# duyhominhnguyen/conan-fgw

Measured on AMD Instinct MI355X. Metric: molecules/s (K=5 conformers), higher is better.
Workload: dtype f32

## Files before the change

### conan-fgw_amd/csrc/filter_fused.hip

```cpp
#include "fp_planes.h"

namespace {

constexpr int GP = 64;
constexpr int W1S = GP + 8;
constexpr int FF_THREADS = 512;

constexpr int FF_NPL = 2;
constexpr int FF_OP = 36;

template <int F, bool CF = false, int NT = FF_THREADS>
__global__ void __launch_bounds__(NT) k_filter_fused(
    const float *__restrict__ dist, const int *__restrict__ num_edges_dev, int max_edges, const float *__restrict__ offset,
    int Gs, float coeff, float cutoff, const float *__restrict__ w1, const float *__restrict__ b1,
    const float *__restrict__ w2, const float *__restrict__ b2, float *__restrict__ Wout, float *__restrict__ h1_out,
    const float *__restrict__ xin = nullptr, const int *__restrict__ col = nullptr, const int *__restrict__ tgt = nullptr) {
    constexpr int MB = F / 32;
    constexpr int W2S = F + 8;
    constexpr int W2WORDS = (FF_NPL * F * W2S) / 2;
    extern __shared__ __attribute__((aligned(16))) float lds[];
    constexpr int W1WORDS = (FF_NPL * F * W1S) / 2;
    float *W1L = lds;
    float *W2L = W1L + W1WORDS;
    float *B1L = W2L + W2WORDS;
    float *B2L = B1L + F;
    float *OFL = B2L + F;
    float *OT = OFL + GP + (threadIdx.x >> 6) * (32 * FF_OP);
    __shared__ float wred[NT / 64];
    float us1 = 1.0f, us2 = 1.0f;
    const int tid = threadIdx.x, lane = tid & 63, wave = tid >> 6;
    const int E = num_edges_dev ? min(*num_edges_dev, max_edges) : max_edges;
    const int tiles = (E + 31) >> 5;
    if (!CF && (int)blockIdx.x * (NT / 64) >= tiles) return;
    if (CF && tiles == 0) return;

    {
        constexpr int PER1 = (F * GP + NT - 1) / NT;
        float wv[PER1];
#pragma unroll
        for (int u = 0; u < PER1; ++u) {
            const int t = tid + u * NT, f = t / GP, k = t - f * GP;
            wv[u] = (t < F * GP && k < Gs) ? w1[(size_t)f * Gs + k] : 0.f;
        }
        float sc1 = 1.0f;
        float am = 0.f;
#pragma unroll
        for (int u = 0; u < PER1; ++u) am = fmaxf(am, fabsf(wv[u]));
        __syncthreads();
        pow2_scale(block_absmax<NT>(am, wred), sc1, us1);
#pragma unroll
        for (int u = 0; u < PER1; ++u) {
            const int t = tid + u * NT, f = t / GP, k = t - f * GP;
            if (t >= F * GP) continue;
            _Float16 *W1H = reinterpret_cast<_Float16 *>(W1L);
            const float v = wv[u] * sc1;
            const _Float16 h1 = (_Float16)v;
            W1H[(0 * F + f) * W1S + k] = h1;
            W1H[(1 * F + f) * W1S + k] = (_Float16)(v - (float)h1);
        }
    }
    {
        constexpr int PER2 = (F * F + NT - 1) / NT;
        float wv[PER2];
#pragma unroll
        for (int u = 0; u < PER2; ++u) { const int t = tid + u * NT; wv[u] = t < F * F ? w2[t] : 0.f; }
        float sc2 = 1.0f;
        float am = 0.f;
#pragma unroll
        for (int u = 0; u < PER2; ++u) am = fmaxf(am, fabsf(wv[u]));
        __syncthreads();
        pow2_scale(block_absmax<NT>(am, wred), sc2, us2);
#pragma unroll
        for (int u = 0; u < PER2; ++u) {
            const int t = tid + u * NT;
            if (t >= F * F) continue;
            const int f2 = t / F, f = t - f2 * F;
            const int kk = f & 15, hh = (kk >> 2) & 1, jj = (kk & 3) + 4 * (kk >> 3);
            const int colp = (f & ~15) + 8 * hh + jj;
            _Float16 *W2H = reinterpret_cast<_Float16 *>(W2L);
            const float v = wv[u] * sc2;
            const _Float16 h1 = (_Float16)v;
            W2H[(0 * F + f2) * W2S + colp] = h1;
            W2H[(1 * F + f2) * W2S + colp] = (_Float16)(v - (float)h1);
        }
    }
    for (int t = tid; t < F; t += NT) { B1L[t] = b1[t]; B2L[t] = b2[t]; }
    for (int t = tid; t < GP; t += NT) OFL[t] = t < Gs ? offset[t] : 0.f;
    __syncthreads();

    const int l31 = lane & 31, h = lane >> 5;
    const int per_wg = CF ? (tiles + (int)gridDim.x - 1) / (int)gridDim.x : 0;
    const int lb = CF ? ((gridDim.x & 7) == 0 ? xcd_contiguous_block((int)blockIdx.x, (int)gridDim.x) : (int)blockIdx.x) : 0;
    const int t_begin = CF ? lb * per_wg + wave : blockIdx.x * (NT / 64) + wave;
    const int t_end = CF ? min(tiles, (lb + 1) * per_wg) : tiles;
    const int wave_stride = CF ? NT / 64 : gridDim.x * (NT / 64);
    for (int tile = t_begin; tile < t_end; tile += wave_stride) {
        const int e = (tile << 5) + l31;
        const bool valid = e < E;
        const float d = valid ? dist[e] : 0.f;
        int src = 0, trg = -1;
        if constexpr (CF) { if (valid) { src = col[e]; trg = tgt[e]; } }

        f32x16 acc1[MB];
#pragma unroll
        for (int mb = 0; mb < MB; ++mb)
#pragma unroll
            for (int r = 0; r < 16; ++r) acc1[mb][r] = 0.f;
        {
#pragma unroll
            for (int s = 0; s < GP / 16; ++s) {
                const int kb = 16 * s + 8 * h;
                const float4 o0 = *reinterpret_cast<const float4 *>(&OFL[kb]), o1 = *reinterpret_cast<const float4 *>(&OFL[kb + 4]);
                const float of[8] = {o0.x, o0.y, o0.z, o0.w, o1.x, o1.y, o1.z, o1.w};
                float rb[8];
#pragma unroll
                for (int j = 0; j < 8; ++j) { const float t0 = d - of[j]; rb[j] = exp_neg_f(coeff * (t0 * t0)); }
                const _Float16 *W1H = reinterpret_cast<const _Float16 *>(W1L);
                f16x8 q1, q2;
                split2h(rb, q1, q2);
#pragma unroll
                for (int mb = 0; mb < MB; ++mb) {
                    const int row = 32 * mb + l31;
                    const f16x8 p1 = *reinterpret_cast<const f16x8 *>(&W1H[(0 * F + row) * W1S + kb]);
                    const f16x8 p2 = *reinterpret_cast<const f16x8 *>(&W1H[(1 * F + row) * W1S + kb]);
                    acc1[mb] = __builtin_amdgcn_mfma_f32_32x32x16_f16(p2, q1, acc1[mb], 0, 0, 0);
                    acc1[mb] = __builtin_amdgcn_mfma_f32_32x32x16_f16(p1, q2, acc1[mb], 0, 0, 0);
                    acc1[mb] = __builtin_amdgcn_mfma_f32_32x32x16_f16(p1, q1, acc1[mb], 0, 0, 0);
                }
                __builtin_amdgcn_sched_barrier(0);
            }
        }
#pragma unroll
        for (int mb = 0; mb < MB; ++mb)
#pragma unroll
            for (int q = 0; q < 4; ++q) {
                const float4 bb = *reinterpret_cast<const float4 *>(&B1L[32 * mb + 8 * q + 4 * h]);
                const float us = us1;
                acc1[mb][4 * q + 0] = ssp_f(fmaf(acc1[mb][4 * q + 0], us, bb.x));
                acc1[mb][4 * q + 1] = ssp_f(fmaf(acc1[mb][4 * q + 1], us, bb.y));
                acc1[mb][4 * q + 2] = ssp_f(fmaf(acc1[mb][4 * q + 2], us, bb.z));
                acc1[mb][4 * q + 3] = ssp_f(fmaf(acc1[mb][4 * q + 3], us, bb.w));
            }
        if (!CF && h1_out) {
            typedef float f4 __attribute__((ext_vector_type(4)));
#pragma unroll
            for (int mb = 0; mb < MB; ++mb) {
#pragma unroll
                for (int q = 0; q < 4; ++q)
                    *reinterpret_cast<float4 *>(&OT[l31 * FF_OP + 8 * q + 4 * h]) =
                        make_float4(acc1[mb][4 * q], acc1[mb][4 * q + 1], acc1[mb][4 * q + 2], acc1[mb][4 * q + 3]);
                wave_lds_fence();
#pragma unroll
                for (int i = 0; i < 4; ++i) {
                    const int r = 8 * i + (lane >> 3), c = 4 * (lane & 7);
                    const float4 o = *reinterpret_cast<const float4 *>(&OT[r * FF_OP + c]);
                    const f4 hv4 = {o.x, o.y, o.z, o.w};
                    if ((tile << 5) + r < E) __builtin_nontemporal_store(hv4, reinterpret_cast<f4 *>(h1_out + (size_t)((tile << 5) + r) * F + 32 * mb + c));
                }
                wave_lds_fence();
            }
        }

        const float C = 0.5f * (cosf(__fdiv_rn(d * 3.14159265358979323846f, cutoff)) + 1.0f);
        constexpr int NG = MB >= 4 ? 2 : MB;
#pragma unroll
        for (int n0 = 0; n0 < MB; n0 += NG) {
            f32x16 acc2[NG];
#pragma unroll
            for (int nb = 0; nb < NG; ++nb)
#pragma unroll
                for (int r = 0; r < 16; ++r) acc2[nb][r] = 0.f;
            float4 xg[CF ? NG : 1][4];
            if constexpr (CF) {
#pragma unroll
                for (int nb = 0; nb < NG; ++nb)
#pragma unroll
                    for (int q = 0; q < 4; ++q)
                        xg[nb][q] = valid ? *reinterpret_cast<const float4 *>(xin + (size_t)src * F + 32 * (n0 + nb) + 8 * q + 4 * h) : make_float4(0.f, 0.f, 0.f, 0.f);
            }
            {
#pragma unroll
                for (int ms = 0; ms < 2 * MB; ++ms) {
                    const int mb = ms >> 1, sgrp = ms & 1;
                    float hv[8];
#pragma unroll
                    for (int j = 0; j < 8; ++j) hv[j] = acc1[mb][8 * sgrp + j];
                    const int colp = 32 * mb + 16 * sgrp + 8 * h;
                    const _Float16 *W2H = reinterpret_cast<const _Float16 *>(W2L);
                    f16x8 q1, q2;
                    split2h(hv, q1, q2);
#pragma unroll
                    for (int nb = 0; nb < NG; ++nb) {
                        const int row = 32 * (n0 + nb) + l31;
                        const f16x8 p1 = *reinterpret_cast<const f16x8 *>(&W2H[(0 * F + row) * W2S + colp]);
                        const f16x8 p2 = *reinterpret_cast<const f16x8 *>(&W2H[(1 * F + row) * W2S + colp]);
                        acc2[nb] = __builtin_amdgcn_mfma_f32_32x32x16_f16(p2, q1, acc2[nb], 0, 0, 0);
                        acc2[nb] = __builtin_amdgcn_mfma_f32_32x32x16_f16(p1, q2, acc2[nb], 0, 0, 0);
                        acc2[nb] = __builtin_amdgcn_mfma_f32_32x32x16_f16(p1, q1, acc2[nb], 0, 0, 0);
                    }
                    __builtin_amdgcn_sched_barrier(0);
                }
            }
#pragma unroll
            for (int nb = 0; nb < NG; ++nb) {
#pragma unroll
                for (int q = 0; q < 4; ++q) {
                    const float4 bb = *reinterpret_cast<const float4 *>(&B2L[32 * (n0 + nb) + 8 * q + 4 * h]);
                    float4 o;
                    const float us = us2;
                    o.x = fmaf(acc2[nb][4 * q + 0], us, bb.x) * C;
                    o.y = fmaf(acc2[nb][4 * q + 1], us, bb.y) * C;
                    o.z = fmaf(acc2[nb][4 * q + 2], us, bb.z) * C;
                    o.w = fmaf(acc2[nb][4 * q + 3], us, bb.w) * C;
                    if constexpr (CF) { o.x *= xg[nb][q].x; o.y *= xg[nb][q].y; o.z *= xg[nb][q].z; o.w *= xg[nb][q].w; }
                    *reinterpret_cast<float4 *>(&OT[l31 * FF_OP + 8 * q + 4 * h]) = o;
                }
                wave_lds_fence();
                if constexpr (CF) {
                    {
                        const int c = lane & 31, r0 = 16 * h;
                        float *ocol = Wout + 32 * (n0 + nb) + c;
                        const int t0 = __shfl(trg, 0, 64), t15 = __shfl(trg, 15, 64), t16 = __shfl(trg, 16, 64);
                        const bool joined = t15 == t16;
                        float accs = 0.f, carry = 0.f;
                        int cur = h ? t16 : t0;
                        bool first = true;
#pragma unroll
                        for (int r = 0; r < 16; ++r) {
                            const int tl = __shfl(trg, r, 64), th = __shfl(trg, 16 + r, 64);
                            const int tr = h ? th : tl;
                            if (tr != cur) {
                                if (h && first && joined) carry = accs;
                                else if (cur >= 0) unsafeAtomicAdd(ocol + (size_t)cur * F, accs);
                                accs = 0.f; cur = tr; first = false;
                            }
                            accs += OT[(r0 + r) * FF_OP + c];
                        }
                        if (h && first && joined) { carry = accs; cur = -1; }
                        const float down = __shfl(carry, (lane & 31) + 32, 64);
                        if (!h && joined) accs += down;
                        if (cur >= 0) unsafeAtomicAdd(ocol + (size_t)cur * F, accs);
                    }
                    wave_lds_fence();
                    continue;
                }
#pragma unroll
                for (int i = 0; i < 4; ++i) {
                    const int r = 8 * i + (lane >> 3), c = 4 * (lane & 7);
                    const float4 o = *reinterpret_cast<const float4 *>(&OT[r * FF_OP + c]);
                    if ((tile << 5) + r < E) *reinterpret_cast<float4 *>(Wout + (size_t)((tile << 5) + r) * F + 32 * (n0 + nb) + c) = o;
                }
                wave_lds_fence();
            }
        }
    }
}

template <int F, int NT>
int launch_nt(const float *dist, const int *num_edges_dev, int max_edges, const float *offset, int Gs, float coeff,
              float cutoff, const float *w1, const float *b1, const float *w2, const float *b2, float *W, float *h1, hipStream_t s) {
    const size_t lds = ((size_t)(FF_NPL * F * W1S) / 2 + (size_t)(FF_NPL * F * (F + 8)) / 2 + 2 * F + GP + (NT / 64) * 32 * FF_OP) * 4;
    (void)hipFuncSetAttribute(reinterpret_cast<const void *>(&k_filter_fused<F, false, NT>), hipFuncAttributeMaxDynamicSharedMemorySize, (int)lds);
    const int tiles = (max_edges + 31) / 32;
    int grid = (tiles + NT / 64 - 1) / (NT / 64);
    if (grid > 256) grid = 256;
    k_filter_fused<F, false, NT><<<grid, NT, lds, s>>>(dist, num_edges_dev, max_edges, offset, Gs, coeff, cutoff, w1, b1, w2, b2, W, h1);
    return hipGetLastError() == hipSuccess ? CONAN_OK : CONAN_E_LAUNCH;
}
template <int F>
int launch(const float *dist, const int *num_edges_dev, int max_edges, const float *offset, int Gs, float coeff,
           float cutoff, const float *w1, const float *b1, const float *w2, const float *b2, float *W, float *h1,
           hipStream_t s) {
    return launch_nt<F, FF_THREADS>(dist, num_edges_dev, max_edges, offset, Gs, coeff, cutoff, w1, b1, w2, b2, W, h1, s);
}

template <int F>
int launch_cf(const float *x, const float *dist, const int *col, const int *tgt, const int *num_edges_dev, int max_edges, const float *offset, int Gs,
              float coeff, float cutoff, const float *w1, const float *b1, const float *w2, const float *b2, int num_atoms, float *out, hipStream_t s) {
    const size_t lds = ((size_t)(FF_NPL * F * W1S) / 2 + (size_t)(FF_NPL * F * (F + 8)) / 2 + 2 * F + GP + (FF_THREADS / 64) * 32 * FF_OP) * 4;
    (void)hipFuncSetAttribute(reinterpret_cast<const void *>(&k_filter_fused<F, true>), hipFuncAttributeMaxDynamicSharedMemorySize, (int)lds);
    if (hipMemsetAsync(out, 0, (size_t)num_atoms * F * sizeof(float), s) != hipSuccess) return CONAN_E_LAUNCH;
    k_filter_fused<F, true><<<256, FF_THREADS, lds, s>>>(dist, num_edges_dev, max_edges, offset, Gs, coeff, cutoff, w1, b1, w2, b2, out, nullptr, x, col, tgt);
    return hipGetLastError() == hipSuccess ? CONAN_OK : CONAN_E_LAUNCH;
}

}

extern "C" {

int conan_filter_cfconv_fwd_supported(int num_gaussians, int num_filters) { return (num_gaussians >= 2 && num_gaussians <= GP && num_filters == 128) ? 1 : 0; }

int conan_filter_cfconv_fwd(const float *x, const float *dist, const int *col, const int *tgt, const int *num_edges_dev, int max_edges,
                            const float *offset, int num_gaussians, float coeff, float cutoff, int num_filters, const float *w1,
                            const float *b1, const float *w2, const float *b2, int num_atoms, float *out, void *stream) {
    if (!x || !dist || !col || !tgt || !offset || !w1 || !b1 || !w2 || !b2 || !out || max_edges < 0 || num_atoms < 0) return CONAN_E_BADARG;
    if (!conan_filter_cfconv_fwd_supported(num_gaussians, num_filters)) return CONAN_E_UNSUPPORTED;
    if (num_atoms == 0) return CONAN_OK;
    hipStream_t s = as_stream(stream);
    if (max_edges == 0) return hipMemsetAsync(out, 0, (size_t)num_atoms * num_filters * sizeof(float), s) == hipSuccess ? CONAN_OK : CONAN_E_LAUNCH;
    return launch_cf<128>(x, dist, col, tgt, num_edges_dev, max_edges, offset, num_gaussians, coeff, cutoff, w1, b1, w2, b2, num_atoms, out, s);
}

int conan_filter_fused_supported(int num_gaussians, int num_filters) {
    return (num_gaussians >= 2 && num_gaussians <= GP && (num_filters == 32 || num_filters == 64 || num_filters == 128)) ? 1 : 0;
}

int conan_filter_fwd(const float *dist, const int *num_edges_dev, int max_edges, const float *offset, int num_gaussians,
                     float coeff, float cutoff, int num_filters, const float *w1, const float *b1, const float *w2,
                     const float *b2, float *W, float *h1_out, void *stream) {
    if (!dist || !offset || !w1 || !b1 || !w2 || !b2 || !W || max_edges < 0) return CONAN_E_BADARG;
    if (!conan_filter_fused_supported(num_gaussians, num_filters)) return CONAN_E_UNSUPPORTED;
    if (max_edges == 0) return CONAN_OK;
    hipStream_t s = as_stream(stream);
#define CONAN_FF(FV) return launch<FV>(dist, num_edges_dev, max_edges, offset, num_gaussians, coeff, cutoff, w1, b1, w2, b2, W, h1_out, s)
    switch (num_filters) {
        case 32: CONAN_FF(32);
        case 64: CONAN_FF(64);
        default: CONAN_FF(128);
    }
#undef CONAN_FF
}

}
```

Before: 117,000.

## Software-pipeline filter kernel: overlap GEMM1, ssp, GEMM2 and next-tile Gaussians

```diff
diff --git a/conan-fgw_amd/csrc/filter_fused.hip b/conan-fgw_amd/csrc/filter_fused.hip
--- a/conan-fgw_amd/csrc/filter_fused.hip
+++ b/conan-fgw_amd/csrc/filter_fused.hip
@@ -1,4 +1,24 @@
 #include "fp_planes.h"
+
+#ifdef CONAN_FF_PROFILE
+static __device__ long long g_ff_prof[8];
+extern "C" int conan_debug_ff_prof(long long *out, int reset) {
+    if (out && hipMemcpyFromSymbol(out, HIP_SYMBOL(g_ff_prof), sizeof(long long) * 8) != hipSuccess) return -2;
+    if (reset) { long long z[8] = {0}; if (hipMemcpyToSymbol(HIP_SYMBOL(g_ff_prof), z, sizeof(z)) != hipSuccess) return -2; }
+    return 0;
+}
+extern "C" const char *conan_debug_ff_prof_names() {
+    return "weight staging|first tile: distance, Gaussians|GEMM1 block 0|ssp(t) + GEMM1(t+1) + GEMM2(t-1) + h1 store(t-1)|"
+           "last block: h1 store, GEMM2, W stores, next Gaussians|last W store|-|-";
+}
+#define FF_PROF_DECL long long prof_t = clock64(); long long prof_acc[8] = {0, 0, 0, 0, 0, 0, 0, 0}
+#define FF_PROF(k) do { const long long t_ = clock64(); prof_acc[k] += t_ - prof_t; prof_t = t_; } while (0)
+#define FF_PROF_FLUSH do { if ((threadIdx.x & 63) == 0) for (int k_ = 0; k_ < 8; ++k_) atomicAdd(reinterpret_cast<unsigned long long *>(&g_ff_prof[k_]), (unsigned long long)prof_acc[k_]); } while (0)
+#else
+#define FF_PROF_DECL
+#define FF_PROF(k)
+#define FF_PROF_FLUSH
+#endif
 
 namespace {
 
@@ -9,7 +29,17 @@
 constexpr int FF_NPL = 2;
 constexpr int FF_OP = 36;
 
-template <int F, bool CF = false, int NT = FF_THREADS>
+typedef unsigned u32x4 __attribute__((ext_vector_type(4)));
+__device__ __forceinline__ __amdgpu_buffer_rsrc_t ff_tile_rows(float *out, int tile, int E, int F) {
+    return __builtin_amdgcn_make_buffer_rsrc(out + (size_t)tile * 32 * F, 0, min(32, E - (tile << 5)) * F * 4, 0x00020000);
+}
+template <bool NTS>
+__device__ __forceinline__ void ff_store4(__amdgpu_buffer_rsrc_t rows, int idx, const float4 &o) {
+    const u32x4 v = {__float_as_uint(o.x), __float_as_uint(o.y), __float_as_uint(o.z), __float_as_uint(o.w)};
+    __builtin_amdgcn_raw_buffer_store_b128(v, rows, idx * 4, 0, NTS ? 2 : 0);
+}
+
+template <int F, bool CF = false, int NT = FF_THREADS, bool H1 = false>
 __global__ void __launch_bounds__(NT) k_filter_fused(
     const float *__restrict__ dist, const int *__restrict__ num_edges_dev, int max_edges, const float *__restrict__ offset,
     int Gs, float coeff, float cutoff, const float *__restrict__ w1, const float *__restrict__ b1,
@@ -33,6 +63,7 @@
     const int tiles = (E + 31) >> 5;
     if (!CF && (int)blockIdx.x * (NT / 64) >= tiles) return;
     if (CF && tiles == 0) return;
+    FF_PROF_DECL;
 
     {
         constexpr int PER1 = (F * GP + NT - 1) / NT;
@@ -87,184 +118,220 @@
     for (int t = tid; t < F; t += NT) { B1L[t] = b1[t]; B2L[t] = b2[t]; }
     for (int t = tid; t < GP; t += NT) OFL[t] = t < Gs ? offset[t] : 0.f;
     __syncthreads();
+    FF_PROF(0);
 
     const int l31 = lane & 31, h = lane >> 5;
+    const _Float16 *W1H = reinterpret_cast<const _Float16 *>(W1L), *W2H = reinterpret_cast<const _Float16 *>(W2L);
+    constexpr bool store_h1 = !CF && H1;
     const int per_wg = CF ? (tiles + (int)gridDim.x - 1) / (int)gridDim.x : 0;
     const int lb = CF ? ((gridDim.x & 7) == 0 ? xcd_contiguous_block((int)blockIdx.x, (int)gridDim.x) : (int)blockIdx.x) : 0;
     const int t_begin = CF ? lb * per_wg + wave : blockIdx.x * (NT / 64) + wave;
     const int t_end = CF ? min(tiles, (lb + 1) * per_wg) : tiles;
     const int wave_stride = CF ? NT / 64 : gridDim.x * (NT / 64);
+
+    constexpr int KS = GP / 16;
+    float d_next = 0.f;
+    int src_next = 0, trg_next = -1;
+    auto request = [&](int tile) {
+        const int e = (tile << 5) + l31;
+        const bool ok = tile < t_end && e < E;
+        d_next = ok ? dist[e] : 0.f;
+        if constexpr (CF) { src_next = ok ? col[e] : 0; trg_next = ok ? tgt[e] : -1; }
+    };
+    f16x8 rq1[KS], rq2[KS];
+    auto gaussians = [&](int s, float d) {
+        const int kb = 16 * s + 8 * h;
+        const float4 o0 = *reinterpret_cast<const float4 *>(&OFL[kb]), o1 = *reinterpret_cast<const float4 *>(&OFL[kb + 4]);
+        const float of[8] = {o0.x, o0.y, o0.z, o0.w, o1.x, o1.y, o1.z, o1.w};
+        float rb[8];
+#pragma unroll
+        for (int j = 0; j < 8; ++j) { const float t0 = d - of[j]; rb[j] = exp_neg_f(coeff * (t0 * t0)); }
+        split2h(rb, rq1[s], rq2[s]);
+    };
+    auto cutoff_factor = [&](float d) { return 0.5f * (cosf(__fdiv_rn(d * 3.14159265358979323846f, cutoff)) + 1.0f); };
+
+    request(t_begin);
+    float d = d_next, C = cutoff_factor(d);
+    int src = src_next, trg = trg_next;
+#pragma unroll
+    for (int s = 0; s < KS; ++s) gaussians(s, d);
+    FF_PROF(1);
+
     for (int tile = t_begin; tile < t_end; tile += wave_stride) {
-        const int e = (tile << 5) + l31;
-        const bool valid = e < E;
-        const float d = valid ? dist[e] : 0.f;
-        int src = 0, trg = -1;
-        if constexpr (CF) { if (valid) { src = col[e]; trg = tgt[e]; } }
-
-        f32x16 acc1[MB];
+        int lane_t = threadIdx.x & 63;
+        asm volatile("" : "+v"(lane_t));
+        const int lane = lane_t, l31 = lane & 31, h = lane >> 5;
+        const bool valid = (tile << 5) + l31 < E;
+        const int tile_s = __builtin_amdgcn_readfirstlane(tile);
+        const __amdgpu_buffer_rsrc_t w_rows = ff_tile_rows(Wout, CF ? 0 : tile_s, CF ? 0 : E, F), h1_rows = ff_tile_rows(h1_out, store_h1 ? tile_s : 0, store_h1 ? E : 0, F);
+        request(tile + wave_stride);
+        f32x16 acc1[MB], acc2[MB];
 #pragma unroll
         for (int mb = 0; mb < MB; ++mb)
 #pragma unroll
-            for (int r = 0; r < 16; ++r) acc1[mb][r] = 0.f;
-        {
-#pragma unroll
-            for (int s = 0; s < GP / 16; ++s) {
-                const int kb = 16 * s + 8 * h;
-                const float4 o0 = *reinterpret_cast<const float4 *>(&OFL[kb]), o1 = *reinterpret_cast<const float4 *>(&OFL[kb + 4]);
-                const float of[8] = {o0.x, o0.y, o0.z, o0.w, o1.x, o1.y, o1.z, o1.w};
-                float rb[8];
-#pragma unroll
-                for (int j = 0; j < 8; ++j) { const float t0 = d - of[j]; rb[j] = exp_neg_f(coeff * (t0 * t0)); }
-                const _Float16 *W1H = reinterpret_cast<const _Float16 *>(W1L);
-                f16x8 q1, q2;
-                split2h(rb, q1, q2);
-#pragma unroll
-                for (int mb = 0; mb < MB; ++mb) {
-                    const int row = 32 * mb + l31;
-                    const f16x8 p1 = *reinterpret_cast<const f16x8 *>(&W1H[(0 * F + row) * W1S + kb]);
-                    const f16x8 p2 = *reinterpret_cast<const f16x8 *>(&W1H[(1 * F + row) * W1S + kb]);
-                    acc1[mb] = __builtin_amdgcn_mfma_f32_32x32x16_f16(p2, q1, acc1[mb], 0, 0, 0);
-                    acc1[mb] = __builtin_amdgcn_mfma_f32_32x32x16_f16(p1, q2, acc1[mb], 0, 0, 0);
-                    acc1[mb] = __builtin_amdgcn_mfma_f32_32x32x16_f16(p1, q1, acc1[mb], 0, 0, 0);
+            for (int r = 0; r < 16; ++r) { acc1[mb][r] = 0.f; acc2[mb][r] = 0.f; }
+
+        auto gemm1_step = [&](int mb, int s) {
+            const int row = 32 * mb + l31, kb = 16 * s + 8 * h;
+            const f16x8 p1 = *reinterpret_cast<const f16x8 *>(&W1H[(0 * F + row) * W1S + kb]);
+            const f16x8 p2 = *reinterpret_cast<const f16x8 *>(&W1H[(1 * F + row) * W1S + kb]);
+            acc1[mb] = __builtin_amdgcn_mfma_f32_32x32x16_f16(p2, rq1[s], acc1[mb], 0, 0, 0);
+            acc1[mb] = __builtin_amdgcn_mfma_f32_32x32x16_f16(p1, rq2[s], acc1[mb], 0, 0, 0);
+            acc1[mb] = __builtin_amdgcn_mfma_f32_32x32x16_f16(p1, rq1[s], acc1[mb], 0, 0, 0);
+        };
+        auto ssp_quarter = [&](int mb, int q) {
+            const float4 bb = *reinterpret_cast<const float4 *>(&B1L[32 * mb + 8 * q + 4 * h]);
+            const float us = us1;
+            acc1[mb][4 * q + 0] = ssp_f(fmaf(acc1[mb][4 * q + 0], us, bb.x));
+            acc1[mb][4 * q + 1] = ssp_f(fmaf(acc1[mb][4 * q + 1], us, bb.y));
+            acc1[mb][4 * q + 2] = ssp_f(fmaf(acc1[mb][4 * q + 2], us, bb.z));
+            acc1[mb][4 * q + 3] = ssp_f(fmaf(acc1[mb][4 * q + 3], us, bb.w));
+        };
+        auto h1_fragment = [&](int ms, f16x8 &q1, f16x8 &q2) {
+            float hv[8];
+#pragma unroll
+            for (int j = 0; j < 8; ++j) hv[j] = acc1[ms >> 1][8 * (ms & 1) + j];
+            split2h(hv, q1, q2);
+        };
+        auto gemm2_step = [&](int nb, int ms, const f16x8 &q1, const f16x8 &q2) {
+            const int row = 32 * nb + l31, colp = 16 * ms + 8 * h;
+            const f16x8 p1 = *reinterpret_cast<const f16x8 *>(&W2H[(0 * F + row) * W2S + colp]);
+            const f16x8 p2 = *reinterpret_cast<const f16x8 *>(&W2H[(1 * F + row) * W2S + colp]);
+            acc2[nb] = __builtin_amdgcn_mfma_f32_32x32x16_f16(p2, q1, acc2[nb], 0, 0, 0);
+            acc2[nb] = __builtin_amdgcn_mfma_f32_32x32x16_f16(p1, q2, acc2[nb], 0, 0, 0);
+            acc2[nb] = __builtin_amdgcn_mfma_f32_32x32x16_f16(p1, q1, acc2[nb], 0, 0, 0);
+        };
+        auto slab_put = [&](int q, const float4 &o) { *reinterpret_cast<float4 *>(&OT[l31 * FF_OP + 8 * q + 4 * h]) = o; };
+        auto h1_put = [&](int mb) {
+            wave_lds_fence();
+#pragma unroll
+            for (int q = 0; q < 4; ++q) slab_put(q, make_float4(acc1[mb][4 * q], acc1[mb][4 * q + 1], acc1[mb][4 * q + 2], acc1[mb][4 * q + 3]));
+        };
+        auto h1_flush = [&](int mb) {
+            wave_lds_fence();
+#pragma unroll
+            for (int i = 0; i < 4; ++i) {
+                const int r = 8 * i + (lane >> 3), c = 4 * (lane & 7);
+                ff_store4<true>(h1_rows, r * F + 32 * mb + c, *reinterpret_cast<const float4 *>(&OT[r * FF_OP + c]));
+            }
+        };
+        float4 xg[CF ? 2 : 1][4];
+        auto gather_x = [&](int nb) {
+#pragma unroll
+            for (int q = 0; q < 4; ++q)
+                xg[nb & 1][q] = valid ? *reinterpret_cast<const float4 *>(xin + (size_t)src * F + 32 * nb + 8 * q + 4 * h) : make_float4(0.f, 0.f, 0.f, 0.f);
+        };
+        auto epilogue = [&](int nb) {
+            wave_lds_fence();
+#pragma unroll
+            for (int q = 0; q < 4; ++q) {
+                const float4 bb = *reinterpret_cast<const float4 *>(&B2L[32 * nb + 8 * q + 4 * h]);
+                float4 o;
+                const float us = us2;
+                o.x = fmaf(acc2[nb][4 * q + 0], us, bb.x) * C;
+                o.y = fmaf(acc2[nb][4 * q + 1], us, bb.y) * C;
+                o.z = fmaf(acc2[nb][4 * q + 2], us, bb.z) * C;
+                o.w = fmaf(acc2[nb][4 * q + 3], us, bb.w) * C;
+                if constexpr (CF) { o.x *= xg[nb & 1][q].x; o.y *= xg[nb & 1][q].y; o.z *= xg[nb & 1][q].z; o.w *= xg[nb & 1][q].w; }
+                slab_put(q, o);
+            }
+            wave_lds_fence();
+            if constexpr (CF) {
+                const int c = lane & 31, r0 = 16 * h;
+                float *ocol = Wout + 32 * nb + c;
+                const int t0 = __shfl(trg, 0, 64), t15 = __shfl(trg, 15, 64), t16 = __shfl(trg, 16, 64);
+                const bool joined = t15 == t16;
+                float accs = 0.f, carry = 0.f;
+                int cur = h ? t16 : t0;
+                bool first = true;
+#pragma unroll
+                for (int r = 0; r < 16; ++r) {
+                    const int tl = __shfl(trg, r, 64), th = __shfl(trg, 16 + r, 64);
+                    const int tr = h ? th : tl;
+                    if (tr != cur) {
+                        if (h && first && joined) carry = accs;
+                        else if (cur >= 0) unsafeAtomicAdd(ocol + (size_t)cur * F, accs);
+                        accs = 0.f; cur = tr; first = false;
+                    }
+                    accs += OT[(r0 + r) * FF_OP + c];
                 }
-                __builtin_amdgcn_sched_barrier(0);
-            }
-        }
-#pragma unroll
-        for (int mb = 0; mb < MB; ++mb)
-#pragma unroll
-            for (int q = 0; q < 4; ++q) {
-                const float4 bb = *reinterpret_cast<const float4 *>(&B1L[32 * mb + 8 * q + 4 * h]);
-                const float us = us1;
-                acc1[mb][4 * q + 0] = ssp_f(fmaf(acc1[mb][4 * q + 0], us, bb.x));
-                acc1[mb][4 * q + 1] = ssp_f(fmaf(acc1[mb][4 * q + 1], us, bb.y));
-                acc1[mb][4 * q + 2] = ssp_f(fmaf(acc1[mb][4 * q + 2], us, bb.z));
-                acc1[mb][4 * q + 3] = ssp_f(fmaf(acc1[mb][4 * q + 3], us, bb.w));
-            }
-        if (!CF && h1_out) {
-            typedef float f4 __attribute__((ext_vector_type(4)));
-#pragma unroll
-            for (int mb = 0; mb < MB; ++mb) {
-#pragma unroll
-                for (int q = 0; q < 4; ++q)
-                    *reinterpret_cast<float4 *>(&OT[l31 * FF_OP + 8 * q + 4 * h]) =
-                        make_float4(acc1[mb][4 * q], acc1[mb][4 * q + 1], acc1[mb][4 * q + 2], acc1[mb][4 * q + 3]);
-                wave_lds_fence();
+                if (h && first && joined) { carry = accs; cur = -1; }
+                const float down = __shfl(carry, (lane & 31) + 32, 64);
+                if (!h && joined) accs += down;
+                if (cur >= 0) unsafeAtomicAdd(ocol + (size_t)cur * F, accs);
+            } else {
 #pragma unroll
                 for (int i = 0; i < 4; ++i) {
                     const int r = 8 * i + (lane >> 3), c = 4 * (lane & 7);
-                    const float4 o = *reinterpret_cast<const float4 *>(&OT[r * FF_OP + c]);
-                    const f4 hv4 = {o.x, o.y, o.z, o.w};
-                    if ((tile << 5) + r < E) __builtin_nontemporal_store(hv4, reinterpret_cast<f4 *>(h1_out + (size_t)((tile << 5) + r) * F + 32 * mb + c));
+                    ff_store4<false>(w_rows, r * F + 32 * nb + c, *reinterpret_cast<const float4 *>(&OT[r * FF_OP + c]));
                 }
-                wave_lds_fence();
-            }
-        }
-
-        const float C = 0.5f * (cosf(__fdiv_rn(d * 3.14159265358979323846f, cutoff)) + 1.0f);
-        constexpr int NG = MB >= 4 ? 2 : MB;
-#pragma unroll
-        for (int n0 = 0; n0 < MB; n0 += NG) {
-            f32x16 acc2[NG];
-#pragma unroll
-            for (int nb = 0; nb < NG; ++nb)
-#pragma unroll
-                for (int r = 0; r < 16; ++r) acc2[nb][r] = 0.f;
-            float4 xg[CF ? NG : 1][4];
-            if constexpr (CF) {
-#pragma unroll
-                for (int nb = 0; nb < NG; ++nb)
-#pragma unroll
-                    for (int q = 0; q < 4; ++q)
-                        xg[nb][q] = valid ? *reinterpret_cast<const float4 *>(xin + (size_t)src * F + 32 * (n0 + nb) + 8 * q + 4 * h) : make_float4(0.f, 0.f, 0.f, 0.f);
-            }
-            {
-#pragma unroll
-                for (int ms = 0; ms < 2 * MB; ++ms) {
-                    const int mb = ms >> 1, sgrp = ms & 1;
-                    float hv[8];
-#pragma unroll
-                    for (int j = 0; j < 8; ++j) hv[j] = acc1[mb][8 * sgrp + j];
-                    const int colp = 32 * mb + 16 * sgrp + 8 * h;
-                    const _Float16 *W2H = reinterpret_cast<const _Float16 *>(W2L);
-                    f16x8 q1, q2;
-                    split2h(hv, q1, q2);
-#pragma unroll
-                    for (int nb = 0; nb < NG; ++nb) {
-                        const int row = 32 * (n0 + nb) + l31;
-                        const f16x8 p1 = *reinterpret_cast<const f16x8 *>(&W2H[(0 * F + row) * W2S + colp]);
-                        const f16x8 p2 = *reinterpret_cast<const f16x8 *>(&W2H[(1 * F + row) * W2S + colp]);
-                        acc2[nb] = __builtin_amdgcn_mfma_f32_32x32x16_f16(p2, q1, acc2[nb], 0, 0, 0);
-                        acc2[nb] = __builtin_amdgcn_mfma_f32_32x32x16_f16(p1, q2, acc2[nb], 0, 0, 0);
-                        acc2[nb] = __builtin_amdgcn_mfma_f32_32x32x16_f16(p1, q1, acc2[nb], 0, 0, 0);
-                    }
-                    __builtin_amdgcn_sched_barrier(0);
+            }
+        };
+
+#pragma unroll
+        for (int s = 0; s < KS; ++s) gemm1_step(0, s);
+        __builtin_amdgcn_sched_barrier(0);
+        FF_PROF(2);
+
+        constexpr int NH = MB >= 2 ? MB / 2 : 1;
+#pragma unroll
+        for (int t = 0; t < MB; ++t) {
+            f16x8 hq1, hq2;
+#pragma unroll
+            for (int i = 0; i < 4; ++i) {
+                if (t + 1 < MB) gemm1_step(t + 1, i);
+                if (t >= 1) {
+                    const int ms = 2 * (t - 1) + (i >> 1);
+                    if ((i & 1) == 0) h1_fragment(ms, hq1, hq2);
+#pragma unroll
+                    for (int nb = (i & 1) * NH; nb < (i & 1) * NH + NH && nb < MB; ++nb) gemm2_step(nb, ms, hq1, hq2);
+                    if (store_h1) { if (i == 0) h1_put(t - 1); else if (i == 1) h1_flush(t - 1); }
                 }
-            }
-#pragma unroll
-            for (int nb = 0; nb < NG; ++nb) {
-#pragma unroll
-                for (int q = 0; q < 4; ++q) {
-                    const float4 bb = *reinterpret_cast<const float4 *>(&B2L[32 * (n0 + nb) + 8 * q + 4 * h]);
-                    float4 o;
-                    const float us = us2;
-                    o.x = fmaf(acc2[nb][4 * q + 0], us, bb.x) * C;
-                    o.y = fmaf(acc2[nb][4 * q + 1], us, bb.y) * C;
-                    o.z = fmaf(acc2[nb][4 * q + 2], us, bb.z) * C;
-                    o.w = fmaf(acc2[nb][4 * q + 3], us, bb.w) * C;
-                    if constexpr (CF) { o.x *= xg[nb][q].x; o.y *= xg[nb][q].y; o.z *= xg[nb][q].z; o.w *= xg[nb][q].w; }
-                    *reinterpret_cast<float4 *>(&OT[l31 * FF_OP + 8 * q + 4 * h]) = o;
+                ssp_quarter(t, i);
+                __builtin_amdgcn_sched_barrier(0);
+            }
+        }
+        FF_PROF(3);
+
+        float C_next = 0.f;
+        {
+            f16x8 fq1[2], fq2[2];
+            h1_fragment(2 * MB - 2, fq1[0], fq2[0]);
+            h1_fragment(2 * MB - 1, fq1[1], fq2[1]);
+#pragma unroll
+            for (int nb = 0; nb < MB; ++nb) {
+                if constexpr (CF) { if (nb >= 1) gather_x(nb - 1); if (nb == MB - 1) gather_x(nb); }
+                gemm2_step(nb, 2 * MB - 2, fq1[0], fq2[0]);
+                gemm2_step(nb, 2 * MB - 1, fq1[1], fq2[1]);
+                if (nb == 0) {
+                    if (store_h1) { h1_put(MB - 1); h1_flush(MB - 1); }
+                    C_next = cutoff_factor(d_next);
+                } else {
+                    epilogue(nb - 1);
                 }
-                wave_lds_fence();
-                if constexpr (CF) {
-                    {
-                        const int c = lane & 31, r0 = 16 * h;
-                        float *ocol = Wout + 32 * (n0 + nb) + c;
-                        const int t0 = __shfl(trg, 0, 64), t15 = __shfl(trg, 15, 64), t16 = __shfl(trg, 16, 64);
-                        const bool joined = t15 == t16;
-                        float accs = 0.f, carry = 0.f;
-                        int cur = h ? t16 : t0;
-                        bool first = true;
-#pragma unroll
-                        for (int r = 0; r < 16; ++r) {
-                            const int tl = __shfl(trg, r, 64), th = __shfl(trg, 16 + r, 64);
-                            const int tr = h ? th : tl;
-                            if (tr != cur) {
-                                if (h && first && joined) carry = accs;
-                                else if (cur >= 0) unsafeAtomicAdd(ocol + (size_t)cur * F, accs);
-                                accs = 0.f; cur = tr; first = false;
-                            }
-                            accs += OT[(r0 + r) * FF_OP + c];
-                        }
-                        if (h && first && joined) { carry = accs; cur = -1; }
-                        const float down = __shfl(carry, (lane & 31) + 32, 64);
-                        if (!h && joined) accs += down;
-                        if (cur >= 0) unsafeAtomicAdd(ocol + (size_t)cur * F, accs);
-                    }
-                    wave_lds_fence();
-                    continue;
-                }
-#pragma unroll
-                for (int i = 0; i < 4; ++i) {
-                    const int r = 8 * i + (lane >> 3), c = 4 * (lane & 7);
-                    const float4 o = *reinterpret_cast<const float4 *>(&OT[r * FF_OP + c]);
-                    if ((tile << 5) + r < E) *reinterpret_cast<float4 *>(Wout + (size_t)((tile << 5) + r) * F + 32 * (n0 + nb) + c) = o;
-                }
-                wave_lds_fence();
-            }
-        }
+#pragma unroll
+                for (int s = nb * KS / MB; s < (nb + 1) * KS / MB; ++s) gaussians(s, d_next);
+                __builtin_amdgcn_sched_barrier(0);
+            }
+        }
+        FF_PROF(4);
+        epilogue(MB - 1);
+        d = d_next; C = C_next; src = src_next; trg = trg_next;
+        FF_PROF(5);
     }
+    FF_PROF_FLUSH;
 }
 
 template <int F, int NT>
 int launch_nt(const float *dist, const int *num_edges_dev, int max_edges, const float *offset, int Gs, float coeff,
               float cutoff, const float *w1, const float *b1, const float *w2, const float *b2, float *W, float *h1, hipStream_t s) {
     const size_t lds = ((size_t)(FF_NPL * F * W1S) / 2 + (size_t)(FF_NPL * F * (F + 8)) / 2 + 2 * F + GP + (NT / 64) * 32 * FF_OP) * 4;
-    (void)hipFuncSetAttribute(reinterpret_cast<const void *>(&k_filter_fused<F, false, NT>), hipFuncAttributeMaxDynamicSharedMemorySize, (int)lds);
+    const auto kernel = h1 ? &k_filter_fused<F, false, NT, true> : &k_filter_fused<F, false, NT, false>;
+    (void)hipFuncSetAttribute(reinterpret_cast<const void *>(kernel), hipFuncAttributeMaxDynamicSharedMemorySize, (int)lds);
     const int tiles = (max_edges + 31) / 32;
     int grid = (tiles + NT / 64 - 1) / (NT / 64);
     if (grid > 256) grid = 256;
-    k_filter_fused<F, false, NT><<<grid, NT, lds, s>>>(dist, num_edges_dev, max_edges, offset, Gs, coeff, cutoff, w1, b1, w2, b2, W, h1);
+    kernel<<<grid, NT, lds, s>>>(dist, num_edges_dev, max_edges, offset, Gs, coeff, cutoff, w1, b1, w2, b2, W, h1, nullptr, nullptr, nullptr);
     return hipGetLastError() == hipSuccess ? CONAN_OK : CONAN_E_LAUNCH;
 }
 template <int F>
```

Measured after the change: 117,000. About the same (-0.0%).
